# CobayaSampler/cobaya

Hardware: AMD Instinct MI355X
Metric: log-posterior evals/sec (whole node), 30-dim gaussian_mixture (higher is better)
Workload: dtype f64

## Files before the change

### cobaya_amd/csrc/capi.hip

```cpp
#include "ctx.h"
#include "host_linalg.h"

int block_slots(const mcmc_hip_ctx* h, int which)
{
    if (!h->blocked) return h->d;
    int L = 0;
    for (size_t b = 0; b < h->blk_size.size(); ++b) {
        if (which == 0) L += h->blk_over[b] * h->blk_size[b];
        else if (which == 1) L += ((int)b <= h->drag_last_slow) ? h->blk_size[b] : 0;
        else L += ((int)b > h->drag_last_slow) ? h->blk_size[b] : 0;
    }
    return L;
}

int upload_constants(mcmc_hip_ctx* h)
{
    if (!h->have_prior || !h->have_target) return MCMC_HIP_OK;
    const int d = h->d, K = h->K;
    const ConstLayout cl{d, K};
    std::vector<double> c((size_t)cl.size() + 16, 0.0);
    for (int i = 0; i < d; ++i) {
        c[cl.lo() + i] = h->lo[i];
        c[cl.hi() + i] = h->hi[i];
        c[cl.loc() + i] = h->loc[i];
// ... 259 lines not shown
    acc(h->dT.resize(d * d + 16));  acc(h->Sg.resize(G * np));
    acc(h->gsum.resize(G * d + np + 1));
    if (r == hipSuccess) {
        h->pooled.p = h->gsum.p + G * d;
        h->acc_total.p = reinterpret_cast<unsigned long long*>(h->gsum.p + G * d + np);
    }
    acc(h->dshift.resize(d));
    if (cfg->emit_capacity > 0) {
        acc(h->rows.resize(W * (size_t)cfg->emit_capacity * (d + 4)));
        acc(h->nrows.resize(W));
    }
    acc(hipHostMalloc((void**)&h->pin_mom, sizeof(double) * (G * d + np + 2), hipHostMallocDefault));
    acc(hipHostMalloc((void**)&h->pin_T, sizeof(double) * 4 * d * d, hipHostMallocDefault));
    for (auto& e : h->pin_T_done) acc(hipEventCreateWithFlags(&e, hipEventDisableTiming));
    acc(hipEventCreateWithFlags(&h->mom_event, hipEventDisableTiming));
    if (h->incremental) {
        int prio_least = 0, prio_greatest = 0;
        acc(hipDeviceGetStreamPriorityRange(&prio_least, &prio_greatest));
        acc(hipStreamCreateWithPriority(&h->stream2, hipStreamNonBlocking, prio_least));
        acc(hipEventCreateWithFlags(&h->mark, hipEventDisableTiming));
        acc(hipEventCreateWithFlags(&h->T_event, hipEventDisableTiming));
        if (const char* e = getenv("MCMC_HIP_EAGER_DIRECTIONS")) h->lazy_dirs = !(e[0] && e[0] != '0');
        if (const char* e = getenv("MCMC_HIP_LOOKAHEAD")) h->lookahead = std::max(1, atoi(e));
        if (const char* e = getenv("MCMC_HIP_DUO")) h->duo = (e[0] && e[0] != '0') ? 1 : 0;
        if (const char* e = getenv("MCMC_HIP_ACCEPT_SLACK")) {
            const double v = strtod(e, nullptr);
            h->accept_slack = v < mcmc::kAcceptSlack ? mcmc::kAcceptSlack : v;
        }
        for (auto& D : h->dirs) acc(hipEventCreateWithFlags(&D.ready, hipEventDisableTiming));
        h->prefetch = !getenv("MCMC_HIP_NO_PREFETCH");
// ... 7 lines not shown
    if (r != hipSuccess) {
        fail(nullptr, MCMC_HIP_ERR_DEVICE, "device allocation failed: %s", hipGetErrorString(r));
        mcmc_hip_destroy(h);
        return MCMC_HIP_ERR_DEVICE;
    }
    *out = h;
    return MCMC_HIP_OK;
}

void mcmc_hip_destroy(mcmc_hip_ctx* h)
{
    if (!h) return;
    (void)hipSetDevice(h->cfg.device);
    if (h->stream) (void)hipStreamSynchronize(h->stream);
    if (h->stream2) (void)hipStreamSynchronize(h->stream2);
    resolve_timing(h);
    for (auto e : h->pool) (void)hipEventDestroy(e);
    for (auto& D : h->dirs) {
        D.V.release(); D.Vf.release(); D.VU.release(); D.vflag.release(); D.vflag_f.release(); D.UU.release();
        D.colflag.release(); D.VW.release(); D.NL.release();
        if (D.ready) (void)hipEventDestroy(D.ready);
    }
    if (h->mark) (void)hipEventDestroy(h->mark);
    if (h->T_event) (void)hipEventDestroy(h->T_event);
    if (h->stream2) (void)hipStreamDestroy(h->stream2);
    h->x.release(); h->logpost.release(); h->logprior.release(); h->loglike.release();
    h->hV.release(); h->hScratch.release(); h->hCols.release();
    h->cblock.release(); h->dT.release(); h->V.release(); h->rows.release(); h->gsum.release();
    h->Sg.release(); h->pooled.p = nullptr;  h->dshift.release(); h->ex.release(); h->elp.release();
    h->ell.release(); h->eder.release(); h->escratch.release(); h->dLrow.release();
    h->dLcol.release(); h->weight_i.release(); h->prej.release();
    h->burn.release(); h->stuck.release(); h->nrows.release(); h->nacc.release();
    h->acc_total.p = nullptr;
    h->dblk.release(); h->vflag.release(); h->vflag_f.release(); h->Vf.release(); h->drag_cs.release();
    for (auto& sl : h->slots)
        if (sl.p) (void)hipHostFree(sl.p);
    h->ck.ring.release(); h->ck.wsum.release(); h->ck.payload.release(); h->ck.ws.release();
    h->ck.out.release(); h->ck.acc_prev.release();
    h->bd.ring.release(); h->bd.bounds.release(); h->bd.payload.release();
    if (h->bd.pin) (void)hipHostFree(h->bd.pin);
// ... 332 lines not shown
    std::vector<double> lp(W), ll(W), lpost(W), xt(W * d);
    int rc = mcmc_hip_evaluate(h, (int)W, x, lp.data(), ll.data(), nullptr);
    if (rc) return rc;
    int bad = 0;
    for (size_t w = 0; w < W; ++w) {
        lpost[w] = lp[w] + ll[w];
        if (!std::isfinite(lpost[w])) ++bad;
        for (size_t i = 0; i < d; ++i) xt[i * W + w] = x[w * d + i];
    }
    if (n_bad) *n_bad = bad;
    if (bad)
        return fail(h, MCMC_HIP_ERR_ARG, "%d initial points have a non-finite log-posterior", bad);
    std::vector<int> ones(W, 1), zeros(W, 0), burn(W, h->cfg.burn_in + 1);
    std::vector<long long> z64(W, 0);
    hipStream_t s = h->stream;
    HIP_TRY(h, hipMemcpyAsync(h->x.p, xt.data(), sizeof(double) * W * d, hipMemcpyHostToDevice, s));
    HIP_TRY(h, hipMemcpyAsync(h->logpost.p, lpost.data(), sizeof(double) * W, hipMemcpyHostToDevice, s));
    HIP_TRY(h, hipMemcpyAsync(h->logprior.p, lp.data(), sizeof(double) * W, hipMemcpyHostToDevice, s));
    HIP_TRY(h, hipMemcpyAsync(h->loglike.p, ll.data(), sizeof(double) * W, hipMemcpyHostToDevice, s));
    HIP_TRY(h, hipMemcpyAsync(h->weight_i.p, ones.data(), sizeof(int) * W, hipMemcpyHostToDevice, s));
    HIP_TRY(h, hipMemcpyAsync(h->prej.p, zeros.data(), sizeof(int) * W, hipMemcpyHostToDevice, s));
    HIP_TRY(h, hipMemcpyAsync(h->burn.p, burn.data(), sizeof(int) * W, hipMemcpyHostToDevice, s));
    HIP_TRY(h, hipMemcpyAsync(h->nacc.p, z64.data(), sizeof(long long) * W, hipMemcpyHostToDevice, s));
    if (h->nrows.p)
        HIP_TRY(h, hipMemcpyAsync(h->nrows.p, zeros.data(), sizeof(int) * W, hipMemcpyHostToDevice, s));
    HIP_TRY(h, hipMemsetAsync(h->stuck.p, 0, sizeof(int), s));
    if (h->fnt.bad.p) HIP_TRY(h, hipMemsetAsync(h->fnt.bad.p, 0, sizeof(int), s));
    HIP_TRY(h, hipMemsetAsync(h->acc_total.p, 0, sizeof(unsigned long long), s));
    if (h->thin_acc.p) HIP_TRY(h, hipMemsetAsync(h->thin_acc.p, 0, sizeof(int) * W, s));
    HIP_TRY(h, hipStreamSynchronize(s));
// ... 45 lines not shown
    return MCMC_HIP_OK;
}

int mcmc_hip_set_full_state(mcmc_hip_ctx* h, const double* x, const double* logpost,
                            const double* logprior, const double* loglike, const int32_t* weight,
                            const int32_t* prior_rej, const int32_t* burn_left,
                            const int64_t* n_accept, uint64_t step)
{
    if (!h) return MCMC_HIP_ERR_ARG;
    if (!h->have_prior || !h->have_target)
        return fail(h, MCMC_HIP_ERR_STATE, "set_prior and set_target_* must precede set_full_state");
    if (!x || !logpost || !logprior || !loglike || !weight || !prior_rej || !burn_left || !n_accept)
        return fail(h, MCMC_HIP_ERR_ARG, "null argument");
    const size_t W = h->W, d = h->d;
    HIP_TRY(h, hipSetDevice(h->cfg.device));
    HIP_TRY(h, hipStreamSynchronize(h->stream));
    std::vector<double> xt(W * d);
    for (size_t w = 0; w < W; ++w) {
        if (!std::isfinite(logpost[w]))
            return fail(h, MCMC_HIP_ERR_ARG, "walker %zu has a non-finite log-posterior", w);
        for (size_t i = 0; i < d; ++i) xt[i * W + w] = x[w * d + i];
    }
    HIP_TRY(h, hipMemcpy(h->x.p, xt.data(), sizeof(double) * W * d, hipMemcpyHostToDevice));
    HIP_TRY(h, hipMemcpy(h->logpost.p, logpost, sizeof(double) * W, hipMemcpyHostToDevice));
    HIP_TRY(h, hipMemcpy(h->logprior.p, logprior, sizeof(double) * W, hipMemcpyHostToDevice));
    HIP_TRY(h, hipMemcpy(h->loglike.p, loglike, sizeof(double) * W, hipMemcpyHostToDevice));
    HIP_TRY(h, hipMemcpy(h->weight_i.p, weight, sizeof(int) * W, hipMemcpyHostToDevice));
    HIP_TRY(h, hipMemcpy(h->prej.p, prior_rej, sizeof(int) * W, hipMemcpyHostToDevice));
    HIP_TRY(h, hipMemcpy(h->burn.p, burn_left, sizeof(int) * W, hipMemcpyHostToDevice));
    HIP_TRY(h, hipMemcpy(h->nacc.p, n_accept, sizeof(int64_t) * W, hipMemcpyHostToDevice));
// ... 76 lines not shown
            if (h->blocked) {
                const int rc = blocked_basis(h, drag ? 1 : 0, c0, ncyc, Lc, dd, h->V, h->vflag, any_1d);
                if (rc != MCMC_HIP_OK) return rc;
            } else {
                HIP_TRY(h, h->V.resize((size_t)n_basis * ncyc * dd));
                mcmc::BasisArgs b{};
                b.T = h->dT.p; b.V = h->V.p;
                b.group0 = basis0;
                b.cycle0 = (uint32_t)c0;
                b.key0 = (uint32_t)h->cfg.seed; b.key1 = (uint32_t)(h->cfg.seed >> 32);
                b.ncyc = ncyc;
                if (h->kb) HIP_TRY(h, h->kb->basis(b, n_basis, h->d, h->stream));
                else HIP_TRY(h, h->k->basis(b, n_basis, h->stream));
            }
        }
        {
            Timed t(h, 0);
            mcmc::StepArgs a{};
            a.x = h->x.p; a.logpost = h->logpost.p; a.logprior = h->logprior.p;
            a.loglike = h->loglike.p; a.weight = h->weight_i.p; a.prior_rej = h->prej.p;
            a.burn_left = h->burn.p; a.n_accept = h->nacc.p; a.stuck = h->stuck.p;
            a.accept_total = h->acc_total.p;
            a.rows = h->rows.p; a.n_rows = h->nrows.p; a.row_cap = h->cfg.emit_capacity;
            a.cblock = h->cblock.p; a.V = h->V.p; a.W = h->W; a.n_modes = h->K;
            a.group_size = h->gs;
            a.norm_mask = h->norm_mask; a.periodic_mask = h->periodic_mask;
            a.walker0 = h->cfg.walker_offset;
            a.key0 = (uint32_t)h->cfg.seed; a.key1 = (uint32_t)(h->cfg.seed >> 32);
            a.step0 = h->step; a.n_steps = n; a.ncyc = ncyc;
            a.uniform_logp = h->uniform_logp; a.temperature = h->cfg.temperature;
// ... 53 lines not shown
            h->n_step_launches += 1;
            take_noted_kernel(h);
        }
        h->step += (unsigned long long)n;
        left -= n;
    }
    return MCMC_HIP_OK;
}

int mcmc_hip_sync(mcmc_hip_ctx* h)
{
    if (!h) return MCMC_HIP_ERR_ARG;
    HIP_TRY(h, hipSetDevice(h->cfg.device));
    HIP_TRY(h, hipStreamSynchronize(h->stream));
    if (h->stream2) HIP_TRY(h, hipStreamSynchronize(h->stream2));
    resolve_timing(h);
    if (h->fnt.on) {
        int bad = 0;
        HIP_TRY(h, hipMemcpy(&bad, h->fnt.bad.p, sizeof(int), hipMemcpyDeviceToHost));
        if (bad) return function_target_error(h, bad);
    }
    int stuck = 0;
    HIP_TRY(h, hipMemcpy(&stuck, h->stuck.p, sizeof(int), hipMemcpyDeviceToHost));
    if (stuck)
        return fail(h, MCMC_HIP_ERR_STUCK,
                    "The chain has been stuck for %g attempts (walker %d), stopping sampling.",
                    h->cfg.max_tries, stuck - 1);
    return MCMC_HIP_OK;
}

// ... 16 lines not shown
    counters[0] = (int64_t)h->step;
    counters[1] = (int64_t)tot;
    counters[2] = stuck;
    counters[3] = dropped;
    return MCMC_HIP_OK;
}

int mcmc_hip_set_moment_shift(mcmc_hip_ctx* h, const double* shift)
{
    if (!h || !shift) return MCMC_HIP_ERR_ARG;
    if (h->n_snapshots != 0)
        return fail(h, MCMC_HIP_ERR_STATE, "the moment shift can only change right after a reset");
    const bool changed = !std::equal(h->shift.begin(), h->shift.end(), shift);
    h->shift.assign(shift, shift + h->d);
    HIP_TRY(h, hipSetDevice(h->cfg.device));
    HIP_TRY(h, hipMemcpyAsync(h->dshift.p, h->shift.data(), sizeof(double) * h->d,
                              hipMemcpyHostToDevice, h->stream));
    if (changed && h->ac.acc.p) {
        h->ac.held = h->ac.head = 0;
        std::fill(h->ac.n_pairs.begin(), h->ac.n_pairs.end(), (int64_t)0);
        HIP_TRY(h, hipMemsetAsync(h->ac.acc.p, 0, sizeof(double) * h->ac.acc.n, h->stream));
    }
    HIP_TRY(h, hipStreamSynchronize(h->stream));
    return MCMC_HIP_OK;
}

int mcmc_hip_accumulate_moments(mcmc_hip_ctx* h)
{
    if (!h) return MCMC_HIP_ERR_ARG;
    if (!h->have_state) return fail(h, MCMC_HIP_ERR_STATE, "no state");
    HIP_TRY(h, hipSetDevice(h->cfg.device));
    Timed t(h, 2);
    mcmc::MomentArgs a{};
    a.x = h->x.p; a.shift = h->dshift.p; a.group_sum = h->gsum.p; a.Sg = h->Sg.p;
    a.pooled = h->pooled.p; a.W = h->W; a.G = h->G;
    if (h->huge) HIP_TRY(h, mcmc_hip_launch_huge_moments(&a, h->gs, h->d, h->stream));
    else if (h->kb) HIP_TRY(h, h->kb->moments(a, h->gs, h->d, h->stream));
    else HIP_TRY(h, h->k->moments(a, h->gs, h->stream));
    h->n_snapshots += 1;
    return MCMC_HIP_OK;
}

int mcmc_hip_read_moments(mcmc_hip_ctx* h, int64_t* n_snapshots, double* group_sum,
                          double* pooled_S, int32_t reset)
{
    if (!h) return MCMC_HIP_ERR_ARG;
    HIP_TRY(h, hipSetDevice(h->cfg.device));
    HIP_TRY(h, hipStreamSynchronize(h->stream));
    if (h->stream2) HIP_TRY(h, hipStreamSynchronize(h->stream2));
    resolve_timing(h);
    const size_t d = h->d, G = h->G, np = d * (d + 1) / 2;
    if (n_snapshots) *n_snapshots = h->n_snapshots;
    if (group_sum)
        HIP_TRY(h, hipMemcpy(group_sum, h->gsum.p, sizeof(double) * G * d, hipMemcpyDeviceToHost));
    if (pooled_S) {
        std::vector<double> p(np);
        HIP_TRY(h, hipMemcpy(p.data(), h->pooled.p, sizeof(double) * np, hipMemcpyDeviceToHost));
        for (size_t i = 0; i < d; ++i)
            for (size_t j = 0; j <= i; ++j)
                pooled_S[i * d + j] = pooled_S[j * d + i] = p[i * (i + 1) / 2 + j];
    }
    if (reset) {
        HIP_TRY(h, hipMemset(h->gsum.p, 0, sizeof(double) * G * d));
        HIP_TRY(h, hipMemset(h->pooled.p, 0, sizeof(double) * np));
        h->n_snapshots = 0;
    }
    return MCMC_HIP_OK;
}

int mcmc_hip_set_moments(mcmc_hip_ctx* h, int64_t n_snapshots, const double* group_sum,
                         const double* pooled_S)
{
    if (!h || !group_sum || !pooled_S || n_snapshots < 0) return MCMC_HIP_ERR_ARG;
    HIP_TRY(h, hipSetDevice(h->cfg.device));
    HIP_TRY(h, hipStreamSynchronize(h->stream));
    const size_t d = h->d, G = h->G, np = d * (d + 1) / 2;
    std::vector<double> p(np);
    for (size_t i = 0; i < d; ++i)
        for (size_t j = 0; j <= i; ++j) p[i * (i + 1) / 2 + j] = pooled_S[i * d + j];
    HIP_TRY(h, hipMemcpy(h->gsum.p, group_sum, sizeof(double) * G * d, hipMemcpyHostToDevice));
    HIP_TRY(h, hipMemcpy(h->pooled.p, p.data(), sizeof(double) * np, hipMemcpyHostToDevice));
    h->n_snapshots = n_snapshots;
    return MCMC_HIP_OK;
}

int mcmc_hip_request_moments(mcmc_hip_ctx* h)
{
    if (!h) return MCMC_HIP_ERR_ARG;
    if (!h->have_state) return fail(h, MCMC_HIP_ERR_STATE, "no state");
    if (h->mom_pending) return fail(h, MCMC_HIP_ERR_STATE, "a moment request is already pending");
    HIP_TRY(h, hipSetDevice(h->cfg.device));
    const size_t d = h->d, G = h->G, np = d * (d + 1) / 2;
    hipStream_t s = h->stream;
    HIP_TRY(h, hipMemcpyAsync(h->pin_mom, h->gsum.p, sizeof(double) * (G * d + np + 1),
                              hipMemcpyDeviceToHost, s));
    HIP_TRY(h, hipMemcpyAsync(h->pin_mom + G * d + np + 1, h->stuck.p, sizeof(int),
                              hipMemcpyDeviceToHost, s));
    if (h->fnt.on)
        HIP_TRY(h, hipMemcpyAsync(reinterpret_cast<int*>(h->pin_mom + G * d + np + 1) + 1, h->fnt.bad.p,
                                  sizeof(int), hipMemcpyDeviceToHost, s));
    h->mom_fn = h->fnt.on;
    if (!h->ck.ring.p) HIP_TRY(h, hipMemsetAsync(h->gsum.p, 0, sizeof(double) * (G * d + np), s));
    HIP_TRY(h, hipEventRecord(h->mom_event, s));
    h->mom_n = h->n_snapshots;
    h->mom_step = h->step;
    h->n_snapshots = 0;
    h->mom_pending = true;
    return MCMC_HIP_OK;
}

int mcmc_hip_fetch_moments(mcmc_hip_ctx* h, int64_t* n_snapshots, double* group_sum,
                           double* pooled_S, int64_t counters[2])
{
    if (!h) return MCMC_HIP_ERR_ARG;
    if (!h->mom_pending) return fail(h, MCMC_HIP_ERR_STATE, "no moment request is pending");
    HIP_TRY(h, hipSetDevice(h->cfg.device));
    HIP_TRY(h, hipEventSynchronize(h->mom_event));
    h->mom_pending = false;
// ... 36 lines not shown
int mcmc_hip_enable_timing(mcmc_hip_ctx* h, int32_t on)
{
    if (!h) return MCMC_HIP_ERR_ARG;
    h->timing = on != 0;
    return MCMC_HIP_OK;
}

uint64_t mcmc_hip_stream_handle(const mcmc_hip_ctx* h) { return h ? (uint64_t)(uintptr_t)h->stream : 0; }

int mcmc_hip_kernel_times(mcmc_hip_ctx* h, double ms[3], int64_t* n_step_launches, int32_t reset)
{
    if (!h || !ms) return MCMC_HIP_ERR_ARG;
    HIP_TRY(h, hipSetDevice(h->cfg.device));
    HIP_TRY(h, hipStreamSynchronize(h->stream));
    if (h->stream2) HIP_TRY(h, hipStreamSynchronize(h->stream2));
    resolve_timing(h);
    for (int i = 0; i < 3; ++i)
        ms[i] = h->n_timed[i] > 0 ? h->ms[i] * ((double)h->n_seen[i] / (double)h->n_timed[i]) : 0.0;
    if (h->bg.on) ms[0] = h->ms[3] + h->ms[4] + h->ms[5];
    if (n_step_launches) *n_step_launches = h->n_step_launches;
    if (reset) {
        for (int i = 0; i < 6; ++i) { h->ms[i] = 0.0; h->n_seen[i] = h->n_timed[i] = 0; }
        h->n_step_launches = 0;
    }
    return MCMC_HIP_OK;
}

int mcmc_hip_binned_kernel_times(mcmc_hip_ctx* h, double ms[3], int64_t n_launches[3], int32_t reset)
{
    if (!h || !ms || !n_launches) return MCMC_HIP_ERR_ARG;
// ... 13 lines not shown
```

### cobaya_amd/csrc/capi_autocorr.hip

```cpp
#include "ctx.h"

namespace {

void ac_release(mcmc_hip_ctx* h)
{
    auto& A = h->ac;
    A.ring.release(); A.ringS.release(); A.Pg.release(); A.acc.release(); A.dims.release();
    if (A.pin) (void)hipHostFree(A.pin);
    A.pin = nullptr;
    A.n = A.lags = A.rows_per_pass = A.held = A.head = 0;
    A.n_pairs.clear(); A.pend_pairs.clear();
    A.pending = false;
}

size_t ac_doubles(const mcmc_hip_ctx* h) { return (size_t)3 * (h->ac.lags + 1) * h->ac.n; }

}

extern "C" {

int mcmc_hip_autocorr_configure(mcmc_hip_ctx* h, int32_t n_dims, const int32_t* dims, int32_t lags)
{
    if (!h) return MCMC_HIP_ERR_ARG;
    if (n_dims < 0) return fail(h, MCMC_HIP_ERR_ARG, "n_dims = %d must be >= 0", n_dims);
// ... 50 lines not shown
    const auto& A = h->ac;
    if (n_dims) *n_dims = A.n;
    if (lags) *lags = A.lags;
    if (n_doubles) *n_doubles = A.acc.p ? (int64_t)ac_doubles(h) : 0;
    if (held) *held = A.held;
    return MCMC_HIP_OK;
}

int mcmc_hip_autocorr_accumulate(mcmc_hip_ctx* h)
{
    if (!h) return MCMC_HIP_ERR_ARG;
    auto& A = h->ac;
    if (!A.acc.p) return fail(h, MCMC_HIP_ERR_STATE, "autocorr_configure must precede autocorr_accumulate");
    if (!h->have_state) return fail(h, MCMC_HIP_ERR_STATE, "no state");
    HIP_TRY(h, hipSetDevice(h->cfg.device));
    const int held = std::min(A.held + 1, A.lags + 1);
    mcmc::AcArgs a{};
    a.x = h->x.p; a.shift = h->dshift.p; a.dims = A.dims.p;
    a.ring = A.ring.p; a.ringS = A.ringS.p; a.Pg = A.Pg.p; a.acc = A.acc.p;
    a.W = h->W; a.G = h->G; a.gs = h->gs; a.n = A.n; a.lags = A.lags;
    a.held = held; a.head = A.head; a.rows_per_pass = A.rows_per_pass;
    HIP_TRY(h, mcmc_hip_launch_autocorr(&a, h->stream));
    A.held = held;
    A.head = (A.head + 1) % (A.lags + 1);
    for (int k = 0; k < held; ++k) A.n_pairs[k] += 1;
    return MCMC_HIP_OK;
}

int mcmc_hip_autocorr_request(mcmc_hip_ctx* h)
{
// ... 60 lines not shown
```

### cobaya_amd/csrc/capi_checkpoint.hip

```cpp
#include "ctx.h"

extern "C" {

int mcmc_hip_checkpoint_set_ring(mcmc_hip_ctx* h, int32_t n_intervals, const double* group_sum,
                                 const double* pooled_S, int32_t min_capacity)
{
    if (!h || n_intervals < 0 || (n_intervals > 0 && (!group_sum || !pooled_S))) return MCMC_HIP_ERR_ARG;
    HIP_TRY(h, hipSetDevice(h->cfg.device));
    HIP_TRY(h, hipStreamSynchronize(h->stream));
    auto& K = h->ck;
    const size_t d = h->d, G = h->G, np = d * (d + 1) / 2, ne = G * d + np;
    int cap = 16;
    while (cap < std::max(n_intervals + 2, (int)min_capacity)) cap *= 2;
    K.ring.release();
    HIP_TRY(h, K.ring.resize((size_t)cap * ne));
    K.cap = cap;
    K.n_done = n_intervals;
    std::vector<double> buf((size_t)std::max(n_intervals, 1) * ne, 0.0);
    for (int k = 0; k < n_intervals; ++k) {
        double* dst = buf.data() + (size_t)k * ne;
        std::copy(group_sum + (size_t)k * G * d, group_sum + (size_t)(k + 1) * G * d, dst);
        const double* S = pooled_S + (size_t)k * d * d;
        for (size_t i = 0; i < d; ++i)
            for (size_t j = 0; j <= i; ++j) dst[G * d + i * (i + 1) / 2 + j] = S[i * d + j];
// ... 32 lines not shown
    if (!K.ring.p) return fail(h, MCMC_HIP_ERR_STATE, "checkpoint_set_ring must precede checkpoint_begin");
    if (K.begun || K.pending) return fail(h, MCMC_HIP_ERR_STATE, "a device checkpoint is already in flight");
    if (!h->mom_pending)
        return fail(h, MCMC_HIP_ERR_STATE, "request_moments (the read-out of this interval) must precede checkpoint_begin");
    if (n_window_intervals < 1 || n_window_intervals > K.cap || n_window_snapshots < 1)
        return fail(h, MCMC_HIP_ERR_ARG, "the window holds %d intervals (ring capacity %d)", n_window_intervals, K.cap);
    HIP_TRY(h, hipSetDevice(h->cfg.device));
    const size_t d = h->d, G = h->G, np = d * (d + 1) / 2, ne = G * d + np;
    mcmc::CkptWindowArgs w{};
    w.acc = h->gsum.p; w.ring = K.ring.p; w.wsum = K.wsum.p; w.n_elem = ne;
    w.means = K.wsum.p + ne; w.n_mean = G * d;
    w.n_per_chain = (double)n_window_snapshots * (double)h->gs;
    w.cap = K.cap; w.slot = (int)(K.n_done % K.cap);
    w.n_slots = n_window_intervals;
    w.first = (int)(((K.n_done - (n_window_intervals - 1)) % K.cap + K.cap) % K.cap);
    HIP_TRY(h, mcmc_hip_launch_ckpt_window(&w, h->stream));
    K.n_done += 1;
    mcmc::CkptPayloadArgs p{};
    p.wsum = K.wsum.p; p.means = K.wsum.p + ne; p.payload = K.payload.p; p.accept_total = h->acc_total.p;
    p.accept_prev = K.acc_prev.p; p.d = (int)d; p.G = (int)G; p.W = h->W;
    p.n_per_chain = (double)n_window_snapshots * (double)h->gs;
    p.steps_since = steps_since;
    HIP_TRY(h, mcmc_hip_launch_ckpt_payload(&p, h->stream));
    if (h->comm) {
        if (int rc = mcmc_comm_allreduce_on_stream(h->comm, K.payload.p, 5 + 2 * d * d + d, 0, h->stream))
            return fail(h, rc, "%s", mcmc_comm_error(h->comm));
    }
    K.begun = true;
    if (payload_device_ptr) *payload_device_ptr = (uint64_t)(uintptr_t)K.payload.p;
    if (payload_len) *payload_len = (int32_t)(5 + 2 * d * d + d);
// ... 73 lines not shown
    const size_t d = h->d, nn = d * d;
    std::copy(K.pin_out, K.pin_out + 8, stats);
    if (mean_of_covs) std::copy(K.pin_out + 8, K.pin_out + 8 + nn, mean_of_covs);
    if (K.pin_out[2] != 0.0) {
        h->cov.assign(K.pin_out + 8, K.pin_out + 8 + nn);
        h->T.assign(K.pin_out + 8 + nn, K.pin_out + 8 + 2 * nn);
        h->have_cov = true;
    }
    return MCMC_HIP_OK;
}

int mcmc_hip_bounds_configure(mcmc_hip_ctx* h, int32_t n_slots)
{
    if (!h || n_slots < 0) return MCMC_HIP_ERR_ARG;
    HIP_TRY(h, hipSetDevice(h->cfg.device));
    HIP_TRY(h, hipStreamSynchronize(h->stream));
    auto& B = h->bd;
    const size_t d = h->d, W = h->W, G = h->G;
    B.ring.release();
    B.n_slots = 0;
    if (n_slots == 0) return MCMC_HIP_OK;
    HIP_TRY(h, B.ring.resize((size_t)n_slots * d * W));
    HIP_TRY(h, B.bounds.resize(G * d * 2));
    HIP_TRY(h, B.payload.resize(1 + 4 * d));
    if (!B.pin) HIP_TRY(h, hipHostMalloc((void**)&B.pin, sizeof(double) * (1 + 4 * d + G * d * 2), hipHostMallocDefault));
    B.n_slots = n_slots;
    return MCMC_HIP_OK;
}

int mcmc_hip_bounds_snapshot(mcmc_hip_ctx* h, int32_t slot)
{
    if (!h) return MCMC_HIP_ERR_ARG;
    auto& B = h->bd;
    if (slot < 0 || slot >= B.n_slots) return fail(h, MCMC_HIP_ERR_ARG, "bounds slot %d of %d", slot, B.n_slots);
    if (!h->have_state) return fail(h, MCMC_HIP_ERR_STATE, "no state");
    HIP_TRY(h, hipSetDevice(h->cfg.device));
    const size_t n = (size_t)h->d * h->W;
    HIP_TRY(h, hipMemcpyAsync(B.ring.p + (size_t)slot * n, h->x.p, sizeof(double) * n,
                              hipMemcpyDeviceToDevice, h->stream));
    return MCMC_HIP_OK;
}

int mcmc_hip_bounds_get_slot(mcmc_hip_ctx* h, int32_t slot, double* x)
{
    if (!h || !x) return MCMC_HIP_ERR_ARG;
    auto& B = h->bd;
    if (slot < 0 || slot >= B.n_slots) return fail(h, MCMC_HIP_ERR_ARG, "bounds slot %d of %d", slot, B.n_slots);
    HIP_TRY(h, hipSetDevice(h->cfg.device));
    HIP_TRY(h, hipStreamSynchronize(h->stream));
    const size_t d = h->d, W = h->W;
    std::vector<double> t(d * W);
    HIP_TRY(h, hipMemcpy(t.data(), B.ring.p + (size_t)slot * d * W, sizeof(double) * d * W, hipMemcpyDeviceToHost));
    for (size_t w = 0; w < W; ++w)
        for (size_t i = 0; i < d; ++i) x[w * d + i] = t[i * W + w];
    return MCMC_HIP_OK;
}

int mcmc_hip_bounds_set_slot(mcmc_hip_ctx* h, int32_t slot, const double* x)
{
    if (!h || !x) return MCMC_HIP_ERR_ARG;
    auto& B = h->bd;
    if (slot < 0 || slot >= B.n_slots) return fail(h, MCMC_HIP_ERR_ARG, "bounds slot %d of %d", slot, B.n_slots);
    HIP_TRY(h, hipSetDevice(h->cfg.device));
    HIP_TRY(h, hipStreamSynchronize(h->stream));
    const size_t d = h->d, W = h->W;
    std::vector<double> t(d * W);
    for (size_t w = 0; w < W; ++w)
        for (size_t i = 0; i < d; ++i) t[i * W + w] = x[w * d + i];
    HIP_TRY(h, hipMemcpy(B.ring.p + (size_t)slot * d * W, t.data(), sizeof(double) * d * W, hipMemcpyHostToDevice));
    return MCMC_HIP_OK;
}

int mcmc_hip_bounds_statistics(mcmc_hip_ctx* h, int32_t n_window, const int32_t* slots, double limfrac,
                               double* stats, double* bounds)
{
    if (!h || !slots || !stats) return MCMC_HIP_ERR_ARG;
    auto& B = h->bd;
    if (B.n_slots == 0) return fail(h, MCMC_HIP_ERR_STATE, "bounds_configure must precede bounds_statistics");
// ... 5 lines not shown
    if ((size_t)n * sizeof(double) > (size_t)mcmc::kBoundsLdsBytes)
        return fail(h, MCMC_HIP_ERR_ARG, "%d snapshots of %d walkers do not fit the LDS of a compute unit", n_window, h->gs);
    HIP_TRY(h, hipSetDevice(h->cfg.device));
    mcmc::CkptBoundsArgs a{};
    a.ring = B.ring.p; a.bounds = B.bounds.p; a.n_slots = n_window; a.d = h->d; a.W = h->W; a.gs = h->gs;
    for (int s = 0; s < n_window; ++s) {
        if (slots[s] < 0 || slots[s] >= B.n_slots) return fail(h, MCMC_HIP_ERR_ARG, "bounds slot %d of %d", slots[s], B.n_slots);
        a.slots[s] = slots[s];
    }
    auto order = [n](double target) {
        long long k = (long long)std::ceil(target) - 1;
        return (int)std::min(std::max(k, 0ll), n - 1);
    };
    a.k_lo = order((double)n * limfrac);
    a.k_hi = order((double)n * (1.0 - limfrac));
    HIP_TRY(h, mcmc_hip_launch_ckpt_bounds(&a, h->G, h->stream));
    mcmc::CkptBoundsReduceArgs r{};
    r.bounds = B.bounds.p; r.shift = h->dshift.p; r.payload = B.payload.p; r.d = h->d; r.G = h->G;
    HIP_TRY(h, mcmc_hip_launch_ckpt_bounds_reduce(&r, h->stream));
    const size_t np_ = 1 + 4 * (size_t)h->d, nb = (size_t)h->G * h->d * 2;
    if (h->comm)
        if (int rc = mcmc_comm_allreduce_on_stream(h->comm, B.payload.p, np_, 0, h->stream))
            return fail(h, rc, "%s", mcmc_comm_error(h->comm));
    HIP_TRY(h, hipMemcpyAsync(B.pin, B.payload.p, sizeof(double) * np_, hipMemcpyDeviceToHost, h->stream));
    if (bounds)
        HIP_TRY(h, hipMemcpyAsync(B.pin + np_, B.bounds.p, sizeof(double) * nb, hipMemcpyDeviceToHost, h->stream));
    HIP_TRY(h, hipStreamSynchronize(h->stream));
    std::copy(B.pin, B.pin + np_, stats);
    if (bounds) std::copy(B.pin + np_, B.pin + np_ + nb, bounds);
    return MCMC_HIP_OK;
// ... 15 lines not shown
```

### cobaya_amd/csrc/capi_incremental.hip

```cpp
#include "ctx.h"

int blocked_basis(mcmc_hip_ctx* h, int which, unsigned long long c0, int ncyc, int L, size_t slab,
                  DevBuf<double>& V, DevBuf<int>& flag, bool& any_1d, hipStream_t st)
{
    if (!st) st = h->stream;
    const int nb = (int)h->blk_size.size();
    any_1d = false;
    for (int b = 0; b < nb; ++b) {
        const bool in_seq = which == 0 || (which == 1) == (b <= h->drag_last_slow);
        any_1d = any_1d || (in_seq && h->blk_size[b] == 1);
    }
    HIP_TRY(h, V.resize((size_t)h->BG * ncyc * slab));
    if (any_1d) HIP_TRY(h, flag.resize((size_t)h->BG * ncyc * L));
    mcmc::BlockedBasisArgs b{};
    b.T = h->dT.p; b.V = V.p; b.vflag = any_1d ? flag.p : nullptr;
    b.block_size = h->dblk.p; b.oversample = h->dblk.p + nb; b.i_of_j = h->dblk.p + 2 * nb;
    b.n_blocks = nb; b.d = h->d; b.which = which; b.drag_last_slow = h->drag_last_slow;
    b.L = L; b.slab = (int)slab;
    b.ld = h->d;
    b.nmax = *std::max_element(h->blk_size.begin(), h->blk_size.end());
    b.group0 = h->cfg.walker_offset / (uint32_t)h->bgs;
    b.cycle0 = (uint32_t)c0;
    b.key0 = (uint32_t)h->cfg.seed; b.key1 = (uint32_t)(h->cfg.seed >> 32);
    b.ncyc = ncyc;
// ... 194 lines not shown
            b.T = h->dT.p; b.V = h->hV.p; b.scratch = h->hScratch.p; b.d = d; b.ncyc = 1;
            b.group0 = h->cfg.walker_offset / (uint32_t)h->bgs; b.cycle0 = (uint32_t)cyc;
            b.key0 = (uint32_t)h->cfg.seed; b.key1 = (uint32_t)(h->cfg.seed >> 32);
            HIP_TRY(h, mcmc_hip_launch_huge_basis(&b, (int)BG, slabs, h->stream));
            h->hV_cycle = cyc; h->hV_epoch = h->dir_epoch;
        }
        {
            Timed t(h, 1);
            HIP_TRY(h, h->hCols.resize(BG * (size_t)n * stride));
            mcmc::HugeDirArgs w{};
            w.V = h->hV.p; w.Lrow = h->inc_Lrow.p; w.prior = h->inc_prior.p; w.out = h->hCols.p;
            w.step0 = h->step; w.cycle0 = cyc; w.n_steps = n; w.ncyc = 1; w.d = d; w.dpad = dpad; w.K = K;
            w.carry_prior = (K == 1 && any_normal) ? 1 : 0;
            HIP_TRY(h, mcmc_hip_launch_huge_dirs(&w, (int)BG, h->stream));
        }
        {
            Timed t(h, 0);
            const ConstLayout cl{d, K};
            mcmc::HugeStepArgs a{};
            a.x = h->x.p; a.y = h->y.p; a.logpost = h->logpost.p; a.logprior = h->logprior.p;
            a.loglike = h->loglike.p; a.weight = h->weight_i.p; a.prior_rej = h->prej.p;
            a.burn_left = h->burn.p; a.n_accept = h->nacc.p; a.accept_total = h->acc_total.p;
            a.stuck = h->stuck.p; a.cols = h->hCols.p; a.prior = h->inc_prior.p;
            a.Lrow = h->inc_Lrow.p; a.mean = h->inc_mean.p; a.scale = h->cblock.p + cl.scale();
            a.cnorm = h->cblock.p + cl.cnorm(); a.mweight = h->cblock.p + cl.weight();
            a.d = d; a.dpad = dpad; a.K = K; a.W = h->W; a.bgs = h->bgs;
            a.walker0 = h->cfg.walker_offset;
            a.key0 = (uint32_t)h->cfg.seed; a.key1 = (uint32_t)(h->cfg.seed >> 32);
            a.step0 = h->step; a.refresh = R; a.n_steps = n;
            a.anchor = h->y_valid ? 0 : 1;
// ... 57 lines not shown
        if (h->periodic[i]) a.periodic_mask4[i >> 5] |= 1u << (i & 31);
    return a;
}

int acquire_direction_set(mcmc_hip_ctx* h, const IncChoice& C, const IncPlan& P, IncSeg& span,
                          bool covers, bool& wait_ready)
{
    auto& D = h->dirs[h->dir_cur];
    if (covers) { span.step0 = D.step0; span.n = D.n; }
    const bool hit = covers ||
        (D.ahead && D.step0 == span.step0 && D.n == span.n && D.epoch == h->dir_epoch);
    if (D.ahead) HIP_TRY(h, hipStreamWaitEvent(h->stream, D.ready, 0));
    D.ahead = false;
    wait_ready = false;
    if (hit) return MCMC_HIP_OK;
    if (h->prefetch && h->lazy_dirs && h->mark_valid && h->stream2) {
        HIP_TRY(h, hipStreamWaitEvent(h->stream2, h->mark, 0));
        if (h->T_fresh) HIP_TRY(h, hipStreamWaitEvent(h->stream2, h->T_event, 0));
        const int rc = make_directions(h, C, P, span, D, h->stream2);
        if (rc != MCMC_HIP_OK) return rc;
        wait_ready = true;
    } else {
        const int rc = make_directions(h, C, P, span, D, h->stream);
        if (rc != MCMC_HIP_OK) return rc;
    }
    h->T_fresh = false;
    return MCMC_HIP_OK;
}

int launch_segment(mcmc_hip_ctx* h, const IncChoice& C, const IncPlan& P, mcmc_hip_ctx::DirSet& D,
                   bool inside, int room, bool& wait_ready, int& n)
{
// ... 3 lines not shown
        if (C.fold && inside) {
            refresh_in_kernel = true;
        } else {
            HIP_TRY(h, mcmc_hip_launch_whiten_state(h->x.p, h->y.p, h->inc_mean.p, h->inc_Lrow.p,
                                                    P.d, h->W, P.K, h->stream));
        }
        h->y_valid = true;
        anchor = true;
    }
    if (C.carry_modes && !h->amode_valid) anchor = true;
    n = plan_segment(P, h->step, room).n;
    if (wait_ready) {
        HIP_TRY(h, hipStreamWaitEvent(h->stream, D.ready, 0));
        wait_ready = false;
    }
    {
        Timed t(h, 0);
        const mcmc::IncStepArgs a =
            fill_inc_args(h, C, P, D, n, (anchor ? 1 : 0) | (refresh_in_kernel ? 2 : 0));
        if (C.carry_modes) h->amode_valid = true;
        HIP_TRY(h, P.launch(&a, h->stream));
        h->n_step_launches += 1;
        take_noted_kernel(h);
    }
    h->step += (unsigned long long)n;
    return MCMC_HIP_OK;
}

int prepare_next_set(mcmc_hip_ctx* h, const IncChoice& C, const IncPlan& P, int left, int n_steps)
{
    auto& N = h->dirs[h->dir_cur ^ 1];
    if (C.fold) {
        HIP_TRY(h, hipEventRecord(h->mark, h->stream));
        h->mark_valid = true;
        const auto& D = h->dirs[h->dir_cur];
        if (h->step < D.step0 + (unsigned long long)D.n) return MCMC_HIP_OK;
        if (h->prefetch && h->stream2 && (left > 0 || !h->lazy_dirs)) {
            const IncSeg nxt = plan_span(
                C, P, h->step, std::max(left, std::min(h->lookahead, 16) * n_steps));
            HIP_TRY(h, hipStreamWaitEvent(h->stream2, h->mark, 0));
            const int rc = make_directions(h, C, P, nxt, N, h->stream2);
            if (rc != MCMC_HIP_OK) return rc;
            N.ahead = true;
        }
    } else if (h->prefetch) {
        const IncSeg nxt = plan_span(C, P, h->step, left > 0 ? left : n_steps);
        HIP_TRY(h, hipEventRecord(h->mark, h->stream));
        h->mark_valid = true;
        if (left > 0 || !h->lazy_dirs) {
            HIP_TRY(h, hipStreamWaitEvent(h->stream2, h->mark, 0));
            const int rc = make_directions(h, C, P, nxt, N, h->stream2);
// ... 242 lines not shown
```

### cobaya_amd/csrc/capi_targets.hip

```cpp
#include "ctx.h"
#include "host_linalg.h"

namespace {

inline int binned_shift(int NT) { return (8 - NT % 8) % 8; }
inline int binned_class(int R, int NT) { return (R + binned_shift(NT)) & 7; }

int binned_chi2(mcmc_hip_ctx* h, const double* delta, double* psum, double* chi2, int n)
{
    auto& B = h->bg;
    mcmc::PlChi2Args c{};
    c.delta = delta; c.Astream = B.Astream.p; c.psum = psum;
    std::memcpy(c.tile_off, B.tile_off, sizeof c.tile_off);
    std::memcpy(c.nk, B.nk, sizeof c.nk);
    c.KT = B.KT; c.ntw = B.ntw; c.n_walkers = n; c.n_sets = n / 64;
    HIP_TRY(h, mcmc_hip_launch_pl_chi2(&c, h->stream));
    if (chi2) HIP_TRY(h, mcmc_hip_launch_pl_combine(psum, chi2, n, h->stream));
    return MCMC_HIP_OK;
}

int binned_residual(mcmc_hip_ctx* h, const double* trial, double* delta, int n)
{
    auto& B = h->bg;
    static const bool scalar = getenv("MCMC_HIP_PL_SCALAR_RESIDUAL") != nullptr;
// ... 84 lines not shown
            Timed t(h, 1);
            HIP_TRY(h, h->V.resize((size_t)h->G * ncyc * dd));
            mcmc::BasisArgs b{};
            b.T = h->dT.p; b.V = h->V.p;
            b.group0 = h->cfg.walker_offset / (uint32_t)h->gs;
            b.cycle0 = (uint32_t)c0;
            b.key0 = (uint32_t)h->cfg.seed; b.key1 = (uint32_t)(h->cfg.seed >> 32);
            b.ncyc = ncyc;
            HIP_TRY(h, h->k->basis(b, h->G, h->stream));
        }
        a.s.V = h->V.p; a.s.ncyc = ncyc;
        for (int s = 0; s < n; ++s) {
            a.s.step0 = h->step;
            a.cyc = (int)(h->step / (unsigned long long)d - c0);
            a.col = (int)(h->step % (unsigned long long)d);
            {
                Timed t(h, 3);
                HIP_TRY(h, mcmc_hip_launch_pl_walker(&a, pending ? 1 : 0, 1, h->stream));
            }
            if (unfused) {
                {
                    Timed t(h, 4);
                    const int rc = binned_residual(h, B.trial.p, B.delta.p, W);
                    if (rc) return rc;
                }
                Timed t(h, 5);
                const int rc = binned_chi2(h, B.delta.p, B.psum.p, nullptr, W);
                if (rc) return rc;
            } else {
                Timed t(h, 5);
// ... 81 lines not shown
            HIP_TRY(h, h->V.resize((size_t)h->G * ncyc * dd));
            mcmc::BasisArgs b{};
            b.T = h->dT.p; b.V = h->V.p;
            b.group0 = h->cfg.walker_offset / (uint32_t)h->gs;
            b.cycle0 = (uint32_t)c0;
            b.key0 = (uint32_t)h->cfg.seed; b.key1 = (uint32_t)(h->cfg.seed >> 32);
            b.ncyc = ncyc;
            if (h->kb) HIP_TRY(h, h->kb->basis(b, h->G, d, h->stream));
            else HIP_TRY(h, h->k->basis(b, h->G, h->stream));
        }
        a.s.V = h->V.p; a.s.ncyc = ncyc;
        for (int s = 0; s < n; ++s) {
            a.s.step0 = h->step;
            a.cyc = (int)(h->step / (unsigned long long)d - c0);
            a.col = (int)(h->step % (unsigned long long)d);
            {
                Timed t(h, 0);
                HIP_TRY(h, mcmc_hip_launch_fn_walker(&a, pending ? 1 : 0, 1, h->stream));
            }
            h->n_step_launches += 1;
            pending = false;
            rc = function_call(h, W, F.points.p, F.ll_t.p);
            if (rc) break;
            pending = true;
            h->step += 1;
        }
        left -= n;
    }
    if (pending) {
        Timed t(h, 0);
// ... 254 lines not shown
```

### cobaya_amd/csrc/ctx.h

```cpp
#pragma once
#include "../../include/mcmc_hip.h"

#include <algorithm>
#include <cmath>
#include <cstdarg>
#include <cstdio>
#include <cstring>
#include <limits>
#include <string>
#include <vector>

#define MCMC_HIP_HOST_SIDE 1
#include "kernels.h"
#include "huge_args.h"
#include "pliklite_args.h"
#include "function_args.h"
#include "checkpoint_args.h"
#include "marginal_args.h"
#include "autocorr_args.h"
#include "comm.h"
#include "inc_choice.h"

MCMC_DECLARE_DIM(1) MCMC_DECLARE_DIM(2) MCMC_DECLARE_DIM(3) MCMC_DECLARE_DIM(4)
MCMC_DECLARE_DIM(5) MCMC_DECLARE_DIM(6) MCMC_DECLARE_DIM(7) MCMC_DECLARE_DIM(8)
// ... 135 lines not shown
        hipEvent_t ready = nullptr;
        bool ahead = false;
        unsigned long long step0 = ~0ull, epoch = 0;
        int n = 0;
    } dirs[2];
    int dir_cur = 0;
    unsigned long long dir_epoch = 0;
    hipStream_t stream2 = nullptr;
    hipEvent_t mark = nullptr;
    bool mark_valid = false;
    bool prefetch = true;
    bool lazy_dirs = true;
    int lookahead = 4;
    int duo = -1;
    double accept_slack = mcmc::kAcceptSlack;
    hipEvent_t T_event = nullptr;
    bool T_fresh = false;
    double* pin_mom = nullptr;
    double* pin_T = nullptr;
    int pin_T_slot = 0;
    hipEvent_t pin_T_done[4] = {nullptr, nullptr, nullptr, nullptr};
    hipEvent_t mom_event = nullptr;
    bool mom_pending = false;
    bool mom_fn = false;
    int64_t mom_n = 0;
    unsigned long long mom_step = 0;
    struct HostSlot { double* p = nullptr; size_t cap_rows = 0; };
    std::vector<HostSlot> slots = std::vector<HostSlot>(4);
    int slot_next = 0;
    DevBuf<double> pack_out;
// ... 149 lines not shown
        }
    }
};

inline void resolve_timing(mcmc_hip_ctx* h)
{
    for (auto& e : h->pending) {
        float ms = 0.f;
        if (hipEventElapsedTime(&ms, e.a, e.b) == hipSuccess) h->ms[e.kind] += ms;
        h->pool.push_back(e.a);
        h->pool.push_back(e.b);
    }
    h->pending.clear();
}

int block_slots(const mcmc_hip_ctx* h, int which);
int upload_constants(mcmc_hip_ctx* h);
int step_binned(mcmc_hip_ctx* h, int n_steps);
int step_function(mcmc_hip_ctx* h, int n_steps);
int evaluate_binned_points(mcmc_hip_ctx* h, int n, const double* x, double* logprior, double* loglike);
int function_call(mcmc_hip_ctx* h, int n, const double* points, double* loglike);
int function_target_error(mcmc_hip_ctx* h, int bad);
int blocked_basis(mcmc_hip_ctx* h, int which, unsigned long long c0, int ncyc, int L, size_t slab,
                  DevBuf<double>& V, DevBuf<int>& flag, bool& any_1d, hipStream_t st = nullptr);
int step_huge(mcmc_hip_ctx* h, int n_steps);
int step_incremental(mcmc_hip_ctx* h, int n_steps);
mcmc::IncChoice inc_choice_of(const mcmc_hip_ctx* h);
```

Baseline: 86.68 billion.

## Add optional side stream for moment snapshots and fix direction prefetch marking

Adds an opt-in third stream, enabled by MCMC_HIP_SNAPSHOT_STREAM, that runs moment accumulation, moment readback and optionally the bounds copy off the main stream. Fork and join events keep ordering, and every writer of x on the main stream joins before launching. The intent is to let snapshot work overlap with the next step kernels. It also changes the incremental fold path so the mark event is recorded only when a new direction span is needed, and allows direction prefetch when only T is fresh. The stream path is off by default, but the prefetch and mark change runs by default.

Result: no change. 87.09 billion (median of 6 runs) (+0.5%).

```diff
diff --git a/cobaya_amd/csrc/capi.hip b/cobaya_amd/csrc/capi.hip
--- a/cobaya_amd/csrc/capi.hip
+++ b/cobaya_amd/csrc/capi.hip
@@ -297,6 +297,16 @@
     acc(hipHostMalloc((void**)&h->pin_T, sizeof(double) * 4 * d * d, hipHostMallocDefault));
     for (auto& e : h->pin_T_done) acc(hipEventCreateWithFlags(&e, hipEventDisableTiming));
     acc(hipEventCreateWithFlags(&h->mom_event, hipEventDisableTiming));
+    {
+        const char* e = getenv("MCMC_HIP_SNAPSHOT_STREAM");
+        const int mode = (e && e[0]) ? atoi(e) : 0;
+        if (mode != 0) {
+            acc(hipStreamCreateWithFlags(&h->stream3, hipStreamNonBlocking));
+            acc(hipEventCreateWithFlags(&h->x_final, hipEventDisableTiming));
+            acc(hipEventCreateWithFlags(&h->snap_done, hipEventDisableTiming));
+            h->bounds_on_snapshot = mode == 2;
+        }
+    }
     if (h->incremental) {
         int prio_least = 0, prio_greatest = 0;
         acc(hipDeviceGetStreamPriorityRange(&prio_least, &prio_greatest));
@@ -334,6 +344,7 @@
     (void)hipSetDevice(h->cfg.device);
     if (h->stream) (void)hipStreamSynchronize(h->stream);
     if (h->stream2) (void)hipStreamSynchronize(h->stream2);
+    if (h->stream3) (void)hipStreamSynchronize(h->stream3);
     resolve_timing(h);
     for (auto e : h->pool) (void)hipEventDestroy(e);
     for (auto& D : h->dirs) {
@@ -344,6 +355,9 @@
     if (h->mark) (void)hipEventDestroy(h->mark);
     if (h->T_event) (void)hipEventDestroy(h->T_event);
     if (h->stream2) (void)hipStreamDestroy(h->stream2);
+    if (h->x_final) (void)hipEventDestroy(h->x_final);
+    if (h->snap_done) (void)hipEventDestroy(h->snap_done);
+    if (h->stream3) (void)hipStreamDestroy(h->stream3);
     h->x.release(); h->logpost.release(); h->logprior.release(); h->loglike.release();
     h->hV.release(); h->hScratch.release(); h->hCols.release();
     h->cblock.release(); h->dT.release(); h->V.release(); h->rows.release(); h->gsum.release();
@@ -706,6 +720,7 @@
     std::vector<int> ones(W, 1), zeros(W, 0), burn(W, h->cfg.burn_in + 1);
     std::vector<long long> z64(W, 0);
     hipStream_t s = h->stream;
+    HIP_TRY(h, snapshot_join(h));
     HIP_TRY(h, hipMemcpyAsync(h->x.p, xt.data(), sizeof(double) * W * d, hipMemcpyHostToDevice, s));
     HIP_TRY(h, hipMemcpyAsync(h->logpost.p, lpost.data(), sizeof(double) * W, hipMemcpyHostToDevice, s));
     HIP_TRY(h, hipMemcpyAsync(h->logprior.p, lp.data(), sizeof(double) * W, hipMemcpyHostToDevice, s));
@@ -781,6 +796,7 @@
         return fail(h, MCMC_HIP_ERR_ARG, "null argument");
     const size_t W = h->W, d = h->d;
     HIP_TRY(h, hipSetDevice(h->cfg.device));
+    HIP_TRY(h, snapshot_join(h));
     HIP_TRY(h, hipStreamSynchronize(h->stream));
     std::vector<double> xt(W * d);
     for (size_t w = 0; w < W; ++w) {
@@ -887,6 +903,7 @@
                 else HIP_TRY(h, h->k->basis(b, n_basis, h->stream));
             }
         }
+        HIP_TRY(h, snapshot_join(h));
         {
             Timed t(h, 0);
             mcmc::StepArgs a{};
@@ -970,6 +987,7 @@
     HIP_TRY(h, hipSetDevice(h->cfg.device));
     HIP_TRY(h, hipStreamSynchronize(h->stream));
     if (h->stream2) HIP_TRY(h, hipStreamSynchronize(h->stream2));
+    if (h->stream3) HIP_TRY(h, hipStreamSynchronize(h->stream3));
     resolve_timing(h);
     if (h->fnt.on) {
         int bad = 0;
@@ -1016,6 +1034,7 @@
     const bool changed = !std::equal(h->shift.begin(), h->shift.end(), shift);
     h->shift.assign(shift, shift + h->d);
     HIP_TRY(h, hipSetDevice(h->cfg.device));
+    HIP_TRY(h, snapshot_join(h));
     HIP_TRY(h, hipMemcpyAsync(h->dshift.p, h->shift.data(), sizeof(double) * h->d,
                               hipMemcpyHostToDevice, h->stream));
     if (changed && h->ac.acc.p) {
@@ -1032,13 +1051,18 @@
     if (!h) return MCMC_HIP_ERR_ARG;
     if (!h->have_state) return fail(h, MCMC_HIP_ERR_STATE, "no state");
     HIP_TRY(h, hipSetDevice(h->cfg.device));
-    Timed t(h, 2);
-    mcmc::MomentArgs a{};
-    a.x = h->x.p; a.shift = h->dshift.p; a.group_sum = h->gsum.p; a.Sg = h->Sg.p;
-    a.pooled = h->pooled.p; a.W = h->W; a.G = h->G;
-    if (h->huge) HIP_TRY(h, mcmc_hip_launch_huge_moments(&a, h->gs, h->d, h->stream));
-    else if (h->kb) HIP_TRY(h, h->kb->moments(a, h->gs, h->d, h->stream));
-    else HIP_TRY(h, h->k->moments(a, h->gs, h->stream));
+    hipStream_t st = nullptr;
+    HIP_TRY(h, snapshot_fork(h, &st));
+    {
+        Timed t(h, 2, st);
+        mcmc::MomentArgs a{};
+        a.x = h->x.p; a.shift = h->dshift.p; a.group_sum = h->gsum.p; a.Sg = h->Sg.p;
+        a.pooled = h->pooled.p; a.W = h->W; a.G = h->G;
+        if (h->huge) HIP_TRY(h, mcmc_hip_launch_huge_moments(&a, h->gs, h->d, st));
+        else if (h->kb) HIP_TRY(h, h->kb->moments(a, h->gs, h->d, st));
+        else HIP_TRY(h, h->k->moments(a, h->gs, st));
+    }
+    HIP_TRY(h, snapshot_close(h));
     h->n_snapshots += 1;
     return MCMC_HIP_OK;
 }
@@ -1048,8 +1072,10 @@
 {
     if (!h) return MCMC_HIP_ERR_ARG;
     HIP_TRY(h, hipSetDevice(h->cfg.device));
+    HIP_TRY(h, snapshot_join(h));
     HIP_TRY(h, hipStreamSynchronize(h->stream));
     if (h->stream2) HIP_TRY(h, hipStreamSynchronize(h->stream2));
+    if (h->stream3) HIP_TRY(h, hipStreamSynchronize(h->stream3));
     resolve_timing(h);
     const size_t d = h->d, G = h->G, np = d * (d + 1) / 2;
     if (n_snapshots) *n_snapshots = h->n_snapshots;
@@ -1075,6 +1101,7 @@
 {
     if (!h || !group_sum || !pooled_S || n_snapshots < 0) return MCMC_HIP_ERR_ARG;
     HIP_TRY(h, hipSetDevice(h->cfg.device));
+    HIP_TRY(h, snapshot_join(h));
     HIP_TRY(h, hipStreamSynchronize(h->stream));
     const size_t d = h->d, G = h->G, np = d * (d + 1) / 2;
     std::vector<double> p(np);
@@ -1093,7 +1120,8 @@
     if (h->mom_pending) return fail(h, MCMC_HIP_ERR_STATE, "a moment request is already pending");
     HIP_TRY(h, hipSetDevice(h->cfg.device));
     const size_t d = h->d, G = h->G, np = d * (d + 1) / 2;
-    hipStream_t s = h->stream;
+    hipStream_t s = nullptr;
+    HIP_TRY(h, snapshot_fork(h, &s));
     HIP_TRY(h, hipMemcpyAsync(h->pin_mom, h->gsum.p, sizeof(double) * (G * d + np + 1),
                               hipMemcpyDeviceToHost, s));
     HIP_TRY(h, hipMemcpyAsync(h->pin_mom + G * d + np + 1, h->stuck.p, sizeof(int),
@@ -1104,6 +1132,7 @@
     h->mom_fn = h->fnt.on;
     if (!h->ck.ring.p) HIP_TRY(h, hipMemsetAsync(h->gsum.p, 0, sizeof(double) * (G * d + np), s));
     HIP_TRY(h, hipEventRecord(h->mom_event, s));
+    HIP_TRY(h, snapshot_close(h));
     h->mom_n = h->n_snapshots;
     h->mom_step = h->step;
     h->n_snapshots = 0;
@@ -1170,6 +1199,7 @@
     HIP_TRY(h, hipSetDevice(h->cfg.device));
     HIP_TRY(h, hipStreamSynchronize(h->stream));
     if (h->stream2) HIP_TRY(h, hipStreamSynchronize(h->stream2));
+    if (h->stream3) HIP_TRY(h, hipStreamSynchronize(h->stream3));
     resolve_timing(h);
     for (int i = 0; i < 3; ++i)
         ms[i] = h->n_timed[i] > 0 ? h->ms[i] * ((double)h->n_seen[i] / (double)h->n_timed[i]) : 0.0;
diff --git a/cobaya_amd/csrc/capi_autocorr.hip b/cobaya_amd/csrc/capi_autocorr.hip
--- a/cobaya_amd/csrc/capi_autocorr.hip
+++ b/cobaya_amd/csrc/capi_autocorr.hip
@@ -88,6 +88,7 @@
     if (!A.acc.p) return fail(h, MCMC_HIP_ERR_STATE, "autocorr_configure must precede autocorr_accumulate");
     if (!h->have_state) return fail(h, MCMC_HIP_ERR_STATE, "no state");
     HIP_TRY(h, hipSetDevice(h->cfg.device));
+    HIP_TRY(h, snapshot_join(h));
     const int held = std::min(A.held + 1, A.lags + 1);
     mcmc::AcArgs a{};
     a.x = h->x.p; a.shift = h->dshift.p; a.dims = A.dims.p;
diff --git a/cobaya_amd/csrc/capi_checkpoint.hip b/cobaya_amd/csrc/capi_checkpoint.hip
--- a/cobaya_amd/csrc/capi_checkpoint.hip
+++ b/cobaya_amd/csrc/capi_checkpoint.hip
@@ -70,6 +70,7 @@
     w.cap = K.cap; w.slot = (int)(K.n_done % K.cap);
     w.n_slots = n_window_intervals;
     w.first = (int)(((K.n_done - (n_window_intervals - 1)) % K.cap + K.cap) % K.cap);
+    HIP_TRY(h, snapshot_join(h));
     HIP_TRY(h, mcmc_hip_launch_ckpt_window(&w, h->stream));
     K.n_done += 1;
     mcmc::CkptPayloadArgs p{};
@@ -173,6 +174,7 @@
 {
     if (!h || n_slots < 0) return MCMC_HIP_ERR_ARG;
     HIP_TRY(h, hipSetDevice(h->cfg.device));
+    HIP_TRY(h, snapshot_join(h));
     HIP_TRY(h, hipStreamSynchronize(h->stream));
     auto& B = h->bd;
     const size_t d = h->d, W = h->W, G = h->G;
@@ -195,8 +197,11 @@
     if (!h->have_state) return fail(h, MCMC_HIP_ERR_STATE, "no state");
     HIP_TRY(h, hipSetDevice(h->cfg.device));
     const size_t n = (size_t)h->d * h->W;
+    hipStream_t st = h->stream;
+    if (h->bounds_on_snapshot) HIP_TRY(h, snapshot_fork(h, &st));
     HIP_TRY(h, hipMemcpyAsync(B.ring.p + (size_t)slot * n, h->x.p, sizeof(double) * n,
-                              hipMemcpyDeviceToDevice, h->stream));
+                              hipMemcpyDeviceToDevice, st));
+    if (h->bounds_on_snapshot) HIP_TRY(h, snapshot_close(h));
     return MCMC_HIP_OK;
 }
 
@@ -206,6 +211,7 @@
     auto& B = h->bd;
     if (slot < 0 || slot >= B.n_slots) return fail(h, MCMC_HIP_ERR_ARG, "bounds slot %d of %d", slot, B.n_slots);
     HIP_TRY(h, hipSetDevice(h->cfg.device));
+    HIP_TRY(h, snapshot_join(h));
     HIP_TRY(h, hipStreamSynchronize(h->stream));
     const size_t d = h->d, W = h->W;
     std::vector<double> t(d * W);
@@ -221,6 +227,7 @@
     auto& B = h->bd;
     if (slot < 0 || slot >= B.n_slots) return fail(h, MCMC_HIP_ERR_ARG, "bounds slot %d of %d", slot, B.n_slots);
     HIP_TRY(h, hipSetDevice(h->cfg.device));
+    HIP_TRY(h, snapshot_join(h));
     HIP_TRY(h, hipStreamSynchronize(h->stream));
     const size_t d = h->d, W = h->W;
     std::vector<double> t(d * W);
@@ -256,6 +263,7 @@
     };
     a.k_lo = order((double)n * limfrac);
     a.k_hi = order((double)n * (1.0 - limfrac));
+    HIP_TRY(h, snapshot_join(h));
     HIP_TRY(h, mcmc_hip_launch_ckpt_bounds(&a, h->G, h->stream));
     mcmc::CkptBoundsReduceArgs r{};
     r.bounds = B.bounds.p; r.shift = h->dshift.p; r.payload = B.payload.p; r.d = h->d; r.G = h->G;
diff --git a/cobaya_amd/csrc/capi_incremental.hip b/cobaya_amd/csrc/capi_incremental.hip
--- a/cobaya_amd/csrc/capi_incremental.hip
+++ b/cobaya_amd/csrc/capi_incremental.hip
@@ -232,6 +232,7 @@
             w.carry_prior = (K == 1 && any_normal) ? 1 : 0;
             HIP_TRY(h, mcmc_hip_launch_huge_dirs(&w, (int)BG, h->stream));
         }
+        HIP_TRY(h, snapshot_join(h));
         {
             Timed t(h, 0);
             const ConstLayout cl{d, K};
@@ -319,8 +320,8 @@
     D.ahead = false;
     wait_ready = false;
     if (hit) return MCMC_HIP_OK;
-    if (h->prefetch && h->lazy_dirs && h->mark_valid && h->stream2) {
-        HIP_TRY(h, hipStreamWaitEvent(h->stream2, h->mark, 0));
+    if (h->prefetch && h->lazy_dirs && (h->mark_valid || h->T_fresh) && h->stream2) {
+        if (h->mark_valid) HIP_TRY(h, hipStreamWaitEvent(h->stream2, h->mark, 0));
         if (h->T_fresh) HIP_TRY(h, hipStreamWaitEvent(h->stream2, h->T_event, 0));
         const int rc = make_directions(h, C, P, span, D, h->stream2);
         if (rc != MCMC_HIP_OK) return rc;
@@ -354,6 +355,7 @@
         HIP_TRY(h, hipStreamWaitEvent(h->stream, D.ready, 0));
         wait_ready = false;
     }
+    HIP_TRY(h, snapshot_join(h));
     {
         Timed t(h, 0);
         const mcmc::IncStepArgs a =
@@ -371,10 +373,13 @@
 {
     auto& N = h->dirs[h->dir_cur ^ 1];
     if (C.fold) {
+        const auto& D = h->dirs[h->dir_cur];
+        if (h->step < D.step0 + (unsigned long long)D.n) {
+            h->mark_valid = false;
+            return MCMC_HIP_OK;
+        }
         HIP_TRY(h, hipEventRecord(h->mark, h->stream));
         h->mark_valid = true;
-        const auto& D = h->dirs[h->dir_cur];
-        if (h->step < D.step0 + (unsigned long long)D.n) return MCMC_HIP_OK;
         if (h->prefetch && h->stream2 && (left > 0 || !h->lazy_dirs)) {
             const IncSeg nxt = plan_span(
                 C, P, h->step, std::max(left, std::min(h->lookahead, 16) * n_steps));
diff --git a/cobaya_amd/csrc/capi_targets.hip b/cobaya_amd/csrc/capi_targets.hip
--- a/cobaya_amd/csrc/capi_targets.hip
+++ b/cobaya_amd/csrc/capi_targets.hip
@@ -122,6 +122,7 @@
             a.s.step0 = h->step;
             a.cyc = (int)(h->step / (unsigned long long)d - c0);
             a.col = (int)(h->step % (unsigned long long)d);
+            HIP_TRY(h, snapshot_join(h));
             {
                 Timed t(h, 3);
                 HIP_TRY(h, mcmc_hip_launch_pl_walker(&a, pending ? 1 : 0, 1, h->stream));
@@ -233,6 +234,7 @@
             a.s.step0 = h->step;
             a.cyc = (int)(h->step / (unsigned long long)d - c0);
             a.col = (int)(h->step % (unsigned long long)d);
+            HIP_TRY(h, snapshot_join(h));
             {
                 Timed t(h, 0);
                 HIP_TRY(h, mcmc_hip_launch_fn_walker(&a, pending ? 1 : 0, 1, h->stream));
diff --git a/cobaya_amd/csrc/ctx.h b/cobaya_amd/csrc/ctx.h
--- a/cobaya_amd/csrc/ctx.h
+++ b/cobaya_amd/csrc/ctx.h
@@ -173,6 +173,11 @@
     int lookahead = 4;
     int duo = -1;
     double accept_slack = mcmc::kAcceptSlack;
+    hipStream_t stream3 = nullptr;
+    hipEvent_t x_final = nullptr;
+    hipEvent_t snap_done = nullptr;
+    bool snap_open = false;
+    bool bounds_on_snapshot = false;
     hipEvent_t T_event = nullptr;
     bool T_fresh = false;
     double* pin_mom = nullptr;
@@ -352,6 +357,30 @@
     h->pending.clear();
 }
 
+inline hipError_t snapshot_fork(mcmc_hip_ctx* h, hipStream_t* st)
+{
+    *st = h->stream;
+    if (!h->stream3) return hipSuccess;
+    hipError_t e = hipEventRecord(h->x_final, h->stream);
+    if (e == hipSuccess) e = hipStreamWaitEvent(h->stream3, h->x_final, 0);
+    if (e == hipSuccess) *st = h->stream3;
+    return e;
+}
+
+inline hipError_t snapshot_close(mcmc_hip_ctx* h)
+{
+    if (!h->stream3) return hipSuccess;
+    h->snap_open = true;
+    return hipEventRecord(h->snap_done, h->stream3);
+}
+
+inline hipError_t snapshot_join(mcmc_hip_ctx* h)
+{
+    if (!h->snap_open) return hipSuccess;
+    h->snap_open = false;
+    return hipStreamWaitEvent(h->stream, h->snap_done, 0);
+}
+
 int block_slots(const mcmc_hip_ctx* h, int which);
 int upload_constants(mcmc_hip_ctx* h);
 int step_binned(mcmc_hip_ctx* h, int n_steps);
```
